# soedinglab/spacedust

Measured on AMD Instinct MI355X. Metric: clustersearch throughput (genome-pairs/s; SW GCUPS alongside), higher is better.
Workload: dtype int16

## Files before the change

### spacedust_amd/csrc/hip/sd_sw.hip

```cpp
#include "sd_common.h"
#include <unistd.h>


#include <algorithm>
#include <cmath>
#include <cstring>
#include <memory>
#include <omp.h>
#include <numeric>

#include "../host/sd_host.h"
#include "sd_sw_pk.h"

namespace {

using sdpk::SwTask;

template <int RT>
__global__ void __launch_bounds__(64)
sw_score_kernel(const SwTask *__restrict__ tasks, uint32_t nTasks, const uint8_t *__restrict__ qRes,
                const int8_t *__restrict__ qBias, const uint8_t *__restrict__ tRes, const int8_t *__restrict__ mat,
                int go, int ge, int32_t *__restrict__ out, uint2 *__restrict__ boundary,
                const uint32_t *__restrict__ order ,
                const int8_t *__restrict__ qProf ) {
// ... 1223 lines not shown
            uint32_t v = count;
            for (uint32_t d = 0; d < nd; d++) {
                *--o = (char) ('0' + v % 10);
                v /= 10;
            }
        }
        out += __shfl(incl, 63, 64);
        if (starts) runStart = base + (uint32_t) (63 - __clzll((long long) starts));
        left = __shfl(c, 63, 64);
    }
    if (lane == 0) {
        if (WRITE) {
            res[i].btOffset = dense[i];
            res[i].flags = (res[i].flags & 0xFF) | (int32_t) (out << 8);
        } else {
            cigLen[i] = out;
        }
    }
}

constexpr double BB_EVAL_EXACT = 1e-290;
struct BestByGroup {
    const uint32_t *groupOf, *groupKey;
    uint32_t nGroups;
    float seqIdThr, covThr;
    int alnLenThr, covMode;
    double evalThr;
    double evalExact;
};
__device__ __forceinline__ float bbCov(uint32_t startPos, uint32_t endPos, uint32_t len) {
    return (float) (min(len, max(startPos, endPos)) - min(startPos, endPos) + 1u) / (float) len;
}
__device__ __forceinline__ bool bbAccepted(const sd_sw_result &r, const BestByGroup &B, uint32_t qL, uint32_t tL) {
    if (r.btLen <= 0 || r.qStart < 0 || r.tStart < 0) return false;
    const float qcov = bbCov((uint32_t) r.qStart, (uint32_t) r.qEnd, qL), dbcov = bbCov((uint32_t) r.tStart, (uint32_t) r.tEnd, tL);
    const float seqId = (float) r.identical / (float) r.btLen;
    bool cov = true;
    if (B.covMode == 0) cov = qcov >= B.covThr && dbcov >= B.covThr;
    else if (B.covMode == 2) cov = qcov >= B.covThr;
    else if (B.covMode == 1) cov = dbcov >= B.covThr;
    return r.evalue <= B.evalThr * (1.0 + 1e-9) && seqId >= B.seqIdThr && cov && r.btLen >= B.alnLenThr;
}
__device__ __forceinline__ unsigned long long bbPack(const sd_sw_result &r, uint32_t tL, uint32_t key) {
    return ((unsigned long long) min((uint32_t) r.score, 0xFFFFFu) << 44) | ((unsigned long long) (0xFFFFu - min(tL, 0xFFFFu)) << 28) |
           (unsigned long long) (0x0FFFFFFFu - min(key, 0x0FFFFFFFu));
}
__global__ void __launch_bounds__(256)
k_best_mark(uint32_t nPairs, const sd_sw_result *__restrict__ res, const uint8_t *__restrict__ ident, const uint32_t *__restrict__ pq,
            const uint32_t *__restrict__ pt, const uint64_t *__restrict__ qOff, const uint64_t *__restrict__ tOff, BestByGroup B,
            unsigned long long *__restrict__ table) {
    const uint32_t i = blockIdx.x * blockDim.x + threadIdx.x;
    if (i >= nPairs || ident[i]) return;
    const uint32_t q = pq[i], t = pt[i];
    const uint32_t qL = (uint32_t) (qOff[q + 1] - qOff[q]), tL = (uint32_t) (tOff[t + 1] - tOff[t]);
    const sd_sw_result r = res[i];
    if (!bbAccepted(r, B, qL, tL)) return;
    atomicMax(&table[(size_t) q * B.nGroups + B.groupOf[t]], bbPack(r, tL, B.groupKey ? B.groupKey[t] : t));
}
__global__ void __launch_bounds__(256)
k_best_keep(uint32_t nPairs, sd_sw_result *__restrict__ res, const uint8_t *__restrict__ ident, const uint32_t *__restrict__ pq,
            const uint32_t *__restrict__ pt, const uint64_t *__restrict__ qOff, const uint64_t *__restrict__ tOff, BestByGroup B,
            const unsigned long long *__restrict__ table, uint64_t *__restrict__ btLen) {
    const uint32_t i = blockIdx.x * blockDim.x + threadIdx.x;
    if (i >= nPairs || ident[i]) return;
    const uint32_t q = pq[i], t = pt[i];
    const uint32_t qL = (uint32_t) (qOff[q + 1] - qOff[q]), tL = (uint32_t) (tOff[t + 1] - tOff[t]);
    const sd_sw_result r = res[i];
    const bool keep = bbAccepted(r, B, qL, tL) &&
                      (r.evalue < B.evalExact || table[(size_t) q * B.nGroups + B.groupOf[t]] == bbPack(r, tL, B.groupKey ? B.groupKey[t] : t));
    if (!keep) {
        res[i].btLen = 0;
        btLen[i] = 0;
    }
}

__global__ void __launch_bounds__(256)
k_accept(uint32_t nPairs, const sd_sw_result *__restrict__ res, const uint8_t *__restrict__ ident, uint8_t *__restrict__ acc) {
    const uint32_t i = blockIdx.x * blockDim.x + threadIdx.x;
    if (i >= nPairs) return;
    const sd_sw_result &r = res[i];
    acc[i] = (ident[i] || (r.btLen > 0 && r.qStart >= 0 && r.tStart >= 0)) ? 1 : 0;
}
__global__ void __launch_bounds__(256)
k_accept_compact(uint32_t nPairs, const sd_sw_result *__restrict__ res, const uint8_t *__restrict__ acc,
                 const uint64_t *__restrict__ pos, sd_sw_result *__restrict__ outRes, uint32_t *__restrict__ outIdx) {
    const uint32_t i = blockIdx.x * blockDim.x + threadIdx.x;
    if (i >= nPairs || !acc[i]) return;
    outRes[pos[i]] = res[i];
    outIdx[pos[i]] = i;
}
#include "sd_scan_sort.h"

template <typename T>
int devExclusiveScan(sd_ctx *ctx, const T *in, uint64_t *out, size_t n) {
    uint64_t *tmp = nullptr;
    SD_HIP(ctx, wsGet(ctx, "al.scantmp", sdScanTmpBytes(n) / sizeof(uint64_t) + 32, &tmp));
    SD_HIP(ctx, (sdScanLaunch<T, ScanSum64, false, uint64_t>(ctx->stream, in, out, n, tmp)));
    return SD_OK;
}
int devInclusiveMax(sd_ctx *ctx, const uint32_t *in, uint32_t *out, size_t n) {
    uint32_t *tmp = nullptr;
    SD_HIP(ctx, wsGet(ctx, "al.scantmp32", sdScanTmpBytes(n) / sizeof(uint32_t) + 32, &tmp));
    SD_HIP(ctx, (sdScanLaunch<uint32_t, ScanMax32, true, uint32_t>(ctx->stream, in, out, n, tmp)));
    return SD_OK;
}

int devSortPairs(sd_ctx *ctx, const uint32_t *kIn, uint32_t *kOut, const uint32_t *vIn, uint32_t *vOut, size_t n, int endBit) {
    if (n == 0) return SD_OK;
    uint32_t *kTmp = nullptr, *vTmp = nullptr, *cnt = nullptr;
    SD_HIP(ctx, wsGet(ctx, "al.sortK", n, &kTmp));
    SD_HIP(ctx, wsGet(ctx, "al.sortV", n, &vTmp));
    SD_HIP(ctx, wsGet(ctx, "al.sortCounts", sdRadixSortCountsBytes() / sizeof(uint32_t), &cnt));
    SD_HIP(ctx, sdRadixSortPairs(ctx->stream, kIn, vIn, kOut, vOut, kTmp, vTmp, (uint32_t) n, 0, endBit, cnt));
    return SD_OK;
}

__global__ void __launch_bounds__(256)
k_bound_need(uint32_t nPairs, const SwTask *__restrict__ tasks, const uint32_t *__restrict__ keys, uint64_t *__restrict__ need) {
    const uint32_t i = blockIdx.x * blockDim.x + threadIdx.x;
    if (i >= nPairs) return;
    uint64_t v = 0;
    if (keys[i] != KEY_INVALID) {
        const uint32_t ci = keys[i] >> 10;
        if (scoreClassIsMulti(ci)) v = 2ull * (uint64_t) tasks[i].tL;
        else if (ci == N_SCORE_CLASSES - 1 && tasks[i].n > 1024) v = (uint64_t) tasks[i].tL;
    }
    need[i] = v;
}
__global__ void __launch_bounds__(256)
k_bound_apply(uint32_t nPairs, SwTask *__restrict__ tasks, const uint64_t *__restrict__ off) {
    const uint32_t i = blockIdx.x * blockDim.x + threadIdx.x;
    if (i >= nPairs) return;
    tasks[i].boundOff = off[i];
}

constexpr uint32_t PAIR_NONE = 0xFFFFFFFFu;
inline bool sdSwQuads() {
    static const bool on = !(getenv("SD_SW_QUADS") && atoi(getenv("SD_SW_QUADS")) == 0);
    return on;
}
inline int sdSwWaves() {
    static const int w = (sdSwQuads() && getenv("SD_SW_WAVES") && atoi(getenv("SD_SW_WAVES")) == 2) ? 2 : 1;
    return w;
}
constexpr int PAIR_QUERY_BITS = 17;
__global__ void __launch_bounds__(256)
k_pair_keys(uint32_t n, const uint32_t *__restrict__ keys, const uint32_t *__restrict__ pairQ, uint32_t *__restrict__ key2) {
    const uint32_t i = blockIdx.x * blockDim.x + threadIdx.x;
    if (i >= n) return;
    const uint32_t k = keys[i];
    key2[i] = k == KEY_INVALID ? 0xFFFFFFFFu : ((k >> 10) << 26) | (pairQ[i] << 9) | ((k & 1023u) >> 1);
}
__global__ void __launch_bounds__(256)
k_pair_heads(uint32_t n, const uint32_t *__restrict__ keyS, uint32_t *__restrict__ headPos) {
    const uint32_t p = blockIdx.x * blockDim.x + threadIdx.x;
    if (p >= n) return;
    const bool head = p == 0 || (keyS[p] >> 9) != (keyS[p - 1] >> 9);
    headPos[p] = head ? p : 0u;
}
__global__ void __launch_bounds__(256)
k_pair_leaders(uint32_t n, const uint32_t *__restrict__ keyS, const uint32_t *__restrict__ runStart, uint8_t *__restrict__ leader, int quads) {
    const uint32_t p = blockIdx.x * blockDim.x + threadIdx.x;
    if (p > n) return;
    uint8_t v = 0;
    if (p < n && (keyS[p] >> 26) < FIRST_INT32_CLASS) {
        const uint32_t o = p - runStart[p];
        v = (o & 1u) == 0 ? 1 : 0;
        if (quads) {
            const bool lastOfRun = p + 1 >= n || (keyS[p + 1] >> 9) != (keyS[p] >> 9);
            const uint32_t pairs = (o + 1 + 1) / 2;
            if (lastOfRun) v += (uint8_t) (((uint32_t) quads - pairs % (uint32_t) quads) % (uint32_t) quads);
        }
    }
    leader[p] = v;
}
__global__ void __launch_bounds__(256)
k_pair_emit(uint32_t n, const uint32_t *__restrict__ keyS, const uint32_t *__restrict__ vals, const uint32_t *__restrict__ runStartOf,
            const uint64_t *__restrict__ pairIdx, uint32_t *__restrict__ order2) {
    const uint32_t p = blockIdx.x * blockDim.x + threadIdx.x;
    if (p >= n || (keyS[p] >> 26) >= FIRST_INT32_CLASS || ((p - runStartOf[p]) & 1u)) return;
    const uint64_t w = pairIdx[p];
    order2[2 * w] = vals[p];
    const bool mate = p + 1 < n && (keyS[p + 1] >> 9) == (keyS[p] >> 9);
    order2[2 * w + 1] = mate ? vals[p + 1] : PAIR_NONE;
}
__global__ void k_pair_bounds(const uint32_t *__restrict__ keyS, uint32_t n, const uint64_t *__restrict__ pairIdx,
                              uint32_t *__restrict__ b, int nb) {
    const int c = threadIdx.x;
    if (c >= nb) return;
    const uint32_t want = (uint32_t) c << 26;
    uint32_t lo = 0, hi = n;
    while (lo < hi) {
        const uint32_t mid = (lo + hi) >> 1;
        if (keyS[mid] < want) lo = mid + 1;
        else hi = mid;
    }
    b[c] = (uint32_t) pairIdx[lo];
}

int devRunScore(sd_ctx *ctx, uint32_t nPairs, const uint32_t *dKeys, const uint32_t *dVals, uint32_t *dKeysSorted,
                uint32_t *dOrder, uint32_t *dBounds, SwTask *dTasks, uint64_t *dScanA, uint64_t *dScanB,
                const sd_seqset *q, const sd_seqset *t, const int8_t *dMat, int go, int ge, int32_t *dOut,
                uint32_t *nValid, const uint32_t *dPairQ ) {
    const unsigned grid = (nPairs + 255) / 256;
    int rc = SD_OK;
    uint32_t *dOrder2 = nullptr, *dPairBounds = nullptr;
    if (dPairQ) {
        uint32_t *dKey2 = nullptr, *dVals2 = nullptr, *dHead = nullptr, *dRunStart = nullptr;
        uint64_t *dPairIdx = nullptr;
        uint8_t *dLeader = nullptr;
        SD_HIP(ctx, wsGet(ctx, "sp.key2", (size_t) nPairs, &dKey2));
        SD_HIP(ctx, wsGet(ctx, "sp.vals2", (size_t) nPairs, &dVals2));
        SD_HIP(ctx, wsGet(ctx, "sp.head", (size_t) nPairs, &dHead));
        SD_HIP(ctx, wsGet(ctx, "sp.runstart", (size_t) nPairs, &dRunStart));
        SD_HIP(ctx, wsGet(ctx, "sp.leader", (size_t) nPairs + 1, &dLeader));
        SD_HIP(ctx, wsGet(ctx, "sp.pairidx", (size_t) nPairs + 1, &dPairIdx));
        const int padPairs = sdSwQuads() ? 2 * sdSwWaves() : 0;
        const size_t order2Cap = (size_t) 2 * (size_t) std::max(padPairs, 2) * nPairs + 8;
        SD_HIP(ctx, wsGet(ctx, "sp.order2", order2Cap, &dOrder2));
        SD_HIP(ctx, hipMemsetAsync(dOrder2, 0xFF, order2Cap * sizeof(uint32_t), ctx->stream));
        SD_HIP(ctx, wsGet(ctx, "sp.bounds", 64, &dPairBounds));
        hipLaunchKernelGGL(k_pair_keys, dim3(grid), dim3(256), 0, ctx->stream, nPairs, dKeys, dPairQ, dKey2);
        rc = devSortPairs(ctx, dKey2, dKeysSorted, dVals, dVals2, nPairs, 32);
        if (rc != SD_OK) return rc;
        dOrder = dVals2;
        hipLaunchKernelGGL(k_pair_heads, dim3(grid), dim3(256), 0, ctx->stream, nPairs, dKeysSorted, dHead);
        rc = devInclusiveMax(ctx, dHead, dRunStart, nPairs);
        if (rc != SD_OK) return rc;
        hipLaunchKernelGGL(k_pair_leaders, dim3((nPairs + 256) / 256), dim3(256), 0, ctx->stream, nPairs, dKeysSorted, dRunStart, dLeader,
                           padPairs);
        rc = devExclusiveScan(ctx, (const uint8_t *) dLeader, dPairIdx, (size_t) nPairs + 1);
        if (rc != SD_OK) return rc;
        hipLaunchKernelGGL(k_pair_emit, dim3(grid), dim3(256), 0, ctx->stream, nPairs, dKeysSorted, dVals2, dRunStart, dPairIdx, dOrder2);
        hipLaunchKernelGGL(k_pair_bounds, dim3(1), dim3(64), 0, ctx->stream, dKeysSorted, nPairs, dPairIdx, dPairBounds,
                           (int) FIRST_INT32_CLASS + 1);
        hipLaunchKernelGGL(k_bounds, dim3(1), dim3(64), 0, ctx->stream, dKeysSorted, nPairs, 1u << 26, dBounds, (int) N_SCORE_CLASSES + 1);
    } else {
        rc = devSortPairs(ctx, dKeys, dKeysSorted, dVals, dOrder, nPairs, 16);
        if (rc != SD_OK) return rc;
        hipLaunchKernelGGL(k_bounds, dim3(1), dim3(64), 0, ctx->stream, dKeysSorted, nPairs, 1024u, dBounds, (int) N_SCORE_CLASSES + 1);
    }
    hipLaunchKernelGGL(k_bound_need, dim3(grid), dim3(256), 0, ctx->stream, nPairs, dTasks, dKeys, dScanA);
    SD_HIP(ctx, hipMemsetAsync(dScanA + nPairs, 0, sizeof(uint64_t), ctx->stream));
    rc = devExclusiveScan(ctx, dScanA, dScanB, (size_t) nPairs + 1);
    if (rc != SD_OK) return rc;
    hipLaunchKernelGGL(k_bound_apply, dim3(grid), dim3(256), 0, ctx->stream, nPairs, dTasks, dScanB);
    uint32_t hb[N_SCORE_CLASSES + 1], hpb[FIRST_INT32_CLASS + 1];
    uint64_t boundTotal = 0;
    if (dPairQ) SD_HIP(ctx, sdD2H(ctx, hpb, dPairBounds, sizeof(hpb)));
    SD_HIP(ctx, sdD2H(ctx, hb, dBounds, sizeof(hb)));
    SD_HIP(ctx, sdD2H(ctx, &boundTotal, dScanB + nPairs, sizeof(uint64_t)));
    SD_HIP(ctx, sdStreamSync(ctx));
    *nValid = hb[N_SCORE_CLASSES];
    uint2 *dBound = nullptr;
    SD_HIP(ctx, wsGet(ctx, "sw.bound", std::max<uint64_t>(boundTotal, 1), &dBound));
    for (uint32_t ci = 0; ci < N_SCORE_CLASSES; ci++) {
        const uint32_t begin = hb[ci], cnt = hb[ci + 1] - hb[ci];
        if (cnt == 0) continue;
        static const char *const pkNames[N_PK_CLASSES] = {"rt4x32", "rt6x32", "rt7x32", "rt8x32", "rt9x32", "rt10x32", "rt11x32", "rt12x32",
                                                          "rt8x64", "rt10x64", "rt12x64", "rt8x64s2", "rt8x64s3", "rt8x64sN"};
        static const char *const i32Names[4] = {"sw_score.rt4", "sw_score.rt8", "sw_score.rt16", "sw_score.rt32"};
        static const bool long32 = !(getenv("SD_SW_LONG32") && atoi(getenv("SD_SW_LONG32")) == 0);
        static const bool useAligned = !(getenv("SD_SW_ALIGNED") && atoi(getenv("SD_SW_ALIGNED")) == 0);
        const bool shared = dPairQ != nullptr && ci < FIRST_INT32_CLASS;
        const int alignedRT = (ci >= 1 && ci < FIRST_NARROW_MULTI) ? (int) ci + 4 : 0;
        const bool aligned = alignedRT > 0 && useAligned && (alignedRT <= 12 || (shared && long32));
        int generalIdx = 0;
        if (ci >= FIRST_NARROW_MULTI && ci < FIRST_WIDE_CLASS) generalIdx = (int) FIRST_MULTI_PK + (int) (ci - FIRST_NARROW_MULTI);
        else if (alignedRT) generalIdx = alignedRT <= 6 ? 1 : (alignedRT <= 12 ? alignedRT - 5 : (alignedRT <= 16 ? 8 : (alignedRT <= 20 ? 9 : 10)));
        char name[48];
        if (aligned) snprintf(name, sizeof(name), "sw_score_pk.a_seg%d", alignedRT);
        else if (ci < FIRST_WIDE_CLASS) snprintf(name, sizeof(name), "sw_score_pk.%s", pkNames[generalIdx]);
        else if (ci < FIRST_INT32_CLASS) snprintf(name, sizeof(name), "sw_score_pk.w_%s", pkNames[ci - FIRST_WIDE_CLASS]);
        else snprintf(name, sizeof(name), "%s", i32Names[ci - FIRST_INT32_CLASS]);
        ProfScope ps(ctx, name);
        const uint32_t *ord = dOrder + begin;
        uint32_t nOrd = cnt;
        if (shared) {
            ord = dOrder2 + 2 * (size_t) hpb[ci];
            nOrd = 2 * (hpb[ci + 1] - hpb[ci]);
        }
#define SD_PK(RT, LW, MULTI, WIDE)                                                                                          \
    do {                                                                                                                   \
        if (shared) launchScorePk<RT, LW, MULTI, WIDE, true>(ctx, dTasks, ord, nOrd, q, t, dMat, go, ge, dOut, dBound);     \
        else launchScorePk<RT, LW, MULTI, WIDE, false>(ctx, dTasks, ord, nOrd, q, t, dMat, go, ge, dOut, dBound);           \
    } while (0)
#define SD_PKA(RT)                                                                                               \
    case RT:                                                                                                     \
        if (shared && quads && sdSwWaves() == 2) launchScorePkAligned<RT, 32, 2, 2>(ctx, dTasks, ord, nOrd, q, t, dMat, go, ge, dOut);  \
        else if (shared && quads && sdSwChain() > 1) launchScorePkChain<RT>(ctx, dTasks, ord, nOrd, q, t, dMat, go, ge, dOut);  \
        else if (shared && quads) launchScorePkAligned<RT, 32, 2>(ctx, dTasks, ord, nOrd, q, t, dMat, go, ge, dOut);  \
        else if (shared) launchScorePkAligned<RT, 32, 1>(ctx, dTasks, ord, nOrd, q, t, dMat, go, ge, dOut);      \
        else launchScorePkAligned<RT, 32, 0>(ctx, dTasks, ord, nOrd, q, t, dMat, go, ge, dOut);                  \
        break;
#define SD_PKA16(SEG)                                                                                            \
    case SEG: launchScorePkAligned<2 * SEG, 16, 1>(ctx, dTasks, ord, nOrd, q, t, dMat, go, ge, dOut); break;
#define SD_PK_CLASS(WIDE, IDX)                                                \
        switch (IDX) {                                                        \
            case 0: SD_PK(4, 32, false, WIDE); break;                         \
            case 1: SD_PK(6, 32, false, WIDE); break;                         \
            case 2: SD_PK(7, 32, false, WIDE); break;                         \
            case 3: SD_PK(8, 32, false, WIDE); break;                         \
            case 4: SD_PK(9, 32, false, WIDE); break;                         \
            case 5: SD_PK(10, 32, false, WIDE); break;                        \
            case 6: SD_PK(11, 32, false, WIDE); break;                        \
            case 7: SD_PK(12, 32, false, WIDE); break;                        \
            case 8: SD_PK(8, 64, false, WIDE); break;                         \
            case 9: SD_PK(10, 64, false, WIDE); break;                        \
            case 10: SD_PK(12, 64, false, WIDE); break;                       \
            default: SD_PK(8, 64, true, WIDE); break;                         \
        }
        static const int lw16Max = getenv("SD_SW_LW16") ? atoi(getenv("SD_SW_LW16")) : (sdSwQuads() ? 0 : 8);
        const bool quads = sdSwQuads();
        if (aligned && shared && alignedRT <= lw16Max) {
            switch (alignedRT) {
                SD_PKA16(5) SD_PKA16(6) SD_PKA16(7) SD_PKA16(8) SD_PKA16(9) SD_PKA16(10) SD_PKA16(11) SD_PKA16(12)
                default: break;
            }
        } else if (aligned) {
            switch (alignedRT) {
                SD_PKA(5) SD_PKA(6) SD_PKA(7) SD_PKA(8) SD_PKA(9) SD_PKA(10) SD_PKA(11) SD_PKA(12) SD_PKA(13) SD_PKA(14)
                SD_PKA(15) SD_PKA(16) SD_PKA(17) SD_PKA(18) SD_PKA(19) SD_PKA(20) SD_PKA(21) SD_PKA(22) SD_PKA(23) SD_PKA(24)
                default: break;
            }
        } else if (ci < FIRST_WIDE_CLASS) {
            SD_PK_CLASS(false, generalIdx)
        } else if (ci < FIRST_INT32_CLASS) {
            SD_PK_CLASS(true, (int) (ci - FIRST_WIDE_CLASS))
        } else {
            switch (ci - FIRST_INT32_CLASS) {
                case 0: launchScoreIdx<4>(ctx, dTasks, ord, cnt, q, t, dMat, go, ge, dOut, dBound); break;
                case 1: launchScoreIdx<8>(ctx, dTasks, ord, cnt, q, t, dMat, go, ge, dOut, dBound); break;
                case 2: launchScoreIdx<16>(ctx, dTasks, ord, cnt, q, t, dMat, go, ge, dOut, dBound); break;
                default: launchScoreIdx<32>(ctx, dTasks, ord, cnt, q, t, dMat, go, ge, dOut, dBound); break;
            }
        }
#undef SD_PKA
#undef SD_PKA16
#undef SD_PK_CLASS
#undef SD_PK
    }
    SD_HIP(ctx, hipGetLastError());
    return SD_OK;
}

__global__ void __launch_bounds__(256)
k_cells(uint32_t nPairs, const SwTask *__restrict__ tasks, const uint32_t *__restrict__ keys, unsigned long long *__restrict__ acc) {
    const uint32_t i = blockIdx.x * blockDim.x + threadIdx.x;
    unsigned long long c = 0;
    if (i < nPairs && keys[i] != KEY_INVALID) c = (unsigned long long) tasks[i].n * (unsigned long long) tasks[i].tL;
#pragma unroll
    for (int off = 32; off >= 1; off >>= 1) c += __shfl_xor(c, off, 64);
    if ((threadIdx.x & 63) == 0 && c) atomicAdd(acc, c);
}

}

int sdFail(sd_ctx *ctx, int code, const char *fmt, ...) {
    char buf[1024];
    va_list ap;
    va_start(ap, fmt);
    vsnprintf(buf, sizeof(buf), fmt, ap);
    va_end(ap);
    if (ctx) ctx->lastError = buf;
    else fprintf(stderr, "spacedust_gpu: %s\n", buf);
    return code;
}

extern "C" {

int sd_ctx_create(int device, sd_ctx **out) { return sd_ctx_create_prio(device, 0, out); }

int sd_ctx_create_prio(int device, int priority, sd_ctx **out) { return sd_ctx_create_masked(device, priority, 0, out); }

int sd_ctx_create_masked(int device, int priority, int reserveCUs, sd_ctx **out) {
    if (out == nullptr) return SD_EINVAL;
    *out = nullptr;
    int count = 0;
    hipError_t e = hipGetDeviceCount(&count);
    if (e != hipSuccess || count <= 0) {
        fprintf(stderr, "spacedust_gpu: no HIP device visible (%s); this library has no CPU fallback\n",
                e != hipSuccess ? hipGetErrorString(e) : "device count 0");
        return SD_ENODEVICE;
    }
    if (device < 0 || device >= count) return SD_EINVAL;
    if (hipSetDevice(device) != hipSuccess) return SD_ENODEVICE;
    sd_ctx *c = new sd_ctx();
    c->device = device;
    int least = 0, greatest = 0;
    (void) hipDeviceGetStreamPriorityRange(&least, &greatest);
    const int prio = priority < 0 ? greatest : (priority > 0 ? least : (least + greatest) / 2);
    hipError_t se = hipSuccess;
    (void) hipGetDeviceProperties(&c->prop, device);
    const int nCU = c->prop.multiProcessorCount;
    if (reserveCUs > 0 && nCU > 0 && reserveCUs < nCU) {
        std::vector<uint32_t> mask((size_t) (nCU + 31) / 32, 0u);
        for (int b = 0; b < nCU - reserveCUs; b++) mask[(size_t) b / 32] |= 1u << (b % 32);
        se = hipExtStreamCreateWithCUMask(&c->stream, (uint32_t) mask.size(), mask.data());
    } else {
        se = hipStreamCreateWithPriority(&c->stream, hipStreamNonBlocking, prio);
    }
    if (se != hipSuccess) {
        delete c;
        return SD_EHIP;
    }
    const char *syncMode = getenv("SD_SYNC");
    const bool spin = syncMode && strcmp(syncMode, "spin") == 0;
    (void) hipEventCreate(&c->evStart);
    (void) hipEventCreate(&c->evStop);
    if (!spin) (void) hipEventCreateWithFlags(&c->evSync, hipEventDisableTiming);
    (void) hipGetDeviceProperties(&c->prop, device);
    *out = c;
    return SD_OK;
}

void sd_ctx_destroy(sd_ctx *ctx) {
    if (!ctx) return;
// ... 278 lines not shown
        }
        tk.segLen = std::max(1, (tk.n + lanes - 1) / lanes);
        tk.slot = i;
        tk.boundOff = 0;
        if (tk.n > 0 && tk.tL > 0) tasks.push_back(tk);
    }
    std::vector<int32_t> h;
    uint64_t cells = 0;
    int rc = runScoreTasks(ctx, tasks, queries, targets, dMat.p, par->gapOpen, par->gapExtend, h, nPairs, &cells);
    if (rc != SD_OK) return rc;
    if (reverse) ctx->cellsRev = cells; else ctx->cellsFwd = cells;
    for (uint32_t i = 0; i < nPairs; i++) {
        int v = h[3 * i], col = h[3 * i + 1], row = h[3 * i + 2];
        out[3 * i] = v;
        if (!reverse) {
            out[3 * i + 1] = col;
            out[3 * i + 2] = row;
        } else {
            out[3 * i + 1] = col < 0 ? -1 : tEnd[i] - col;
            out[3 * i + 2] = row;
        }
    }
    return SD_OK;
}

static int alignBatchImpl(sd_ctx *ctx, const sd_sw_params *par, const sd_seqset *queries, const sd_seqset *targets,
                          uint32_t nPairs, const uint32_t *pairQ, const uint32_t *pairT, const uint8_t *isIdentity,
                          sd_sw_result *out, char *btPool, uint64_t btCap, uint64_t *btUsed, uint32_t *compactIdx,
                          uint32_t *nCompact, const uint16_t *pairDiag = nullptr ,
                          const float *bestBy = nullptr ) {
    if (!ctx || !par || !queries || !targets || !out) return SD_EINVAL;
    if (compactIdx && (!nCompact || par->swMode != 2)) return sdFail(ctx, SD_EINVAL, "the compact variants need swMode 2 (records with backtraces)");
    (void) hipSetDevice(ctx->device);
    sdD2HReset(ctx);
    if (btUsed) *btUsed = 0;
    if (nCompact) *nCompact = 0;
    if (nPairs == 0) return SD_OK;
    const int go = par->gapOpen, ge = par->gapExtend;
    ctx->cellsFwd = ctx->cellsRev = ctx->cellsTb = 0;
    sd::Evaluer ev;
    sd::initEvaluer(ev, par->dbResidues);
    int matMin = 0;
    for (int i = 0; i < 441; i++) matMin = std::min(matMin, (int) par->matrix[i]);
    for (uint32_t i = 0; i < nPairs; i++)
        if (pairQ[i] >= queries->n || pairT[i] >= targets->n) return sdFail(ctx, SD_EINVAL, "pair %u out of range", i);
    if (targets->dProf) return sdFail(ctx, SD_EUNSUPPORTED, "profile targets are not implemented (profile queries are)");
    std::unique_ptr<HostScope> hs(new HostScope(ctx, "align.upload"));
    DevGateParams gp;
    gp.go = go; gp.ge = ge; gp.matMin = matMin; gp.swMode = par->swMode; gp.covMode = par->covMode; gp.covThr = par->covThr;
    {
        int matMax = 0;
        for (int x = 0; x < 441; x++) matMax = std::max(matMax, (int) par->matrix[x]);
        const int maxEntry = std::max(1, queries->dProf ? queries->maxEntryAdd : matMax + queries->maxEntryAdd);
        gp.wideRowLimit = 32767 / maxEntry;
    }
    gp.evalThr = par->evalThr;
    gp.lambda = ev.lambda; gp.K = ev.K; gp.aI = ev.aI; gp.bI = ev.bI; gp.alphaI = ev.alphaI; gp.betaI = ev.betaI;
    gp.aJ = ev.aJ; gp.bJ = ev.bJ; gp.alphaJ = ev.alphaJ; gp.betaJ = ev.betaJ; gp.sigma = ev.sigma; gp.tau = ev.tau;
    gp.viThr = ev.viThr; gp.vjThr = ev.vjThr; gp.cThr = ev.cThr; gp.dbResidues = ev.dbResidues;

    const size_t N = nPairs;
    const unsigned grid = (unsigned) ((N + 255) / 256);
    int8_t *dMat = nullptr;
    uint32_t *dPQ = nullptr, *dPT = nullptr, *dKeys = nullptr, *dVals = nullptr, *dKeysS = nullptr, *dOrder = nullptr,
             *dBounds = nullptr, *dFwdKeys = nullptr, *dRevKeys = nullptr;
    uint8_t *dIdent = nullptr, *dWord = nullptr;
    int32_t *dMinBias = nullptr, *dOut32 = nullptr, *dOut16 = nullptr, *dOutRev = nullptr, *dTbRes = nullptr;
    int *dErr = nullptr;
    SwTask *dTasks = nullptr;
    TbTask *dTb = nullptr;
    sd_sw_result *dRes = nullptr;
    uint64_t *dScanA = nullptr, *dScanB = nullptr, *dDirBytes = nullptr, *dDirOff = nullptr, *dBtBytes = nullptr,
             *dBtOff = nullptr, *dBtLen = nullptr, *dDense = nullptr;
    unsigned long long *dCells = nullptr;
    SD_HIP(ctx, wsGet(ctx, "al.mat", 448, &dMat));
    SD_HIP(ctx, wsGet(ctx, "al.pq", N, &dPQ));
    SD_HIP(ctx, wsGet(ctx, "al.pt", N, &dPT));
    SD_HIP(ctx, wsGet(ctx, "al.ident", N, &dIdent));
    SD_HIP(ctx, wsGet(ctx, "al.word", N, &dWord));
    SD_HIP(ctx, wsGet(ctx, "al.keys", N, &dKeys));
    SD_HIP(ctx, wsGet(ctx, "al.vals", N, &dVals));
    SD_HIP(ctx, wsGet(ctx, "al.keyss", N, &dKeysS));
    SD_HIP(ctx, wsGet(ctx, "al.order", N, &dOrder));
    SD_HIP(ctx, wsGet(ctx, "al.fwdkeys", N, &dFwdKeys));
    SD_HIP(ctx, wsGet(ctx, "al.revkeys", N, &dRevKeys));
    SD_HIP(ctx, wsGet(ctx, "al.bounds", 64, &dBounds));
    SD_HIP(ctx, wsGet(ctx, "al.minbias", queries->n, &dMinBias));
    SD_HIP(ctx, wsGet(ctx, "al.out32", N * 3, &dOut32));
    SD_HIP(ctx, wsGet(ctx, "al.out16", N * 3, &dOut16));
    SD_HIP(ctx, wsGet(ctx, "al.outrev", N * 3, &dOutRev));
    SD_HIP(ctx, wsGet(ctx, "al.tbres", N * 2, &dTbRes));
    SD_HIP(ctx, wsGet(ctx, "al.err", 4, &dErr));
    SD_HIP(ctx, wsGet(ctx, "al.tasks", N, &dTasks));
    SD_HIP(ctx, wsGet(ctx, "al.tb", N, &dTb));
    SD_HIP(ctx, wsGet(ctx, "al.res", N, &dRes));
    SD_HIP(ctx, wsGet(ctx, "al.scana", N + 1, &dScanA));
    SD_HIP(ctx, wsGet(ctx, "al.scanb", N + 1, &dScanB));
    SD_HIP(ctx, wsGet(ctx, "al.dirbytes", N + 1, &dDirBytes));
    SD_HIP(ctx, wsGet(ctx, "al.diroff", N + 1, &dDirOff));
    SD_HIP(ctx, wsGet(ctx, "al.btbytes", N + 1, &dBtBytes));
    SD_HIP(ctx, wsGet(ctx, "al.btoff", N + 1, &dBtOff));
    SD_HIP(ctx, wsGet(ctx, "al.btlen", N + 1, &dBtLen));
    SD_HIP(ctx, wsGet(ctx, "al.dense", N + 1, &dDense));
    SD_HIP(ctx, wsGet(ctx, "al.cells", 4, &dCells));
    SD_HIP(ctx, hipMemcpyAsync(dMat, par->matrix, 441, hipMemcpyHostToDevice, ctx->stream));
    SD_HIP(ctx, hipMemcpyAsync(dPQ, pairQ, N * sizeof(uint32_t), hipMemcpyHostToDevice, ctx->stream));
    SD_HIP(ctx, hipMemcpyAsync(dPT, pairT, N * sizeof(uint32_t), hipMemcpyHostToDevice, ctx->stream));
    if (isIdentity) SD_HIP(ctx, hipMemcpyAsync(dIdent, isIdentity, N, hipMemcpyHostToDevice, ctx->stream));
    else SD_HIP(ctx, hipMemsetAsync(dIdent, 0, N, ctx->stream));
    SD_HIP(ctx, hipMemcpyAsync(dMinBias, queries->dProf ? queries->hProfBias.data() : queries->hMinBias.data(),
                               queries->n * sizeof(int32_t), hipMemcpyHostToDevice, ctx->stream));
    SD_HIP(ctx, hipMemsetAsync(dErr, 0, 4 * sizeof(int), ctx->stream));
    SD_HIP(ctx, hipMemsetAsync(dCells, 0, 4 * sizeof(unsigned long long), ctx->stream));
    SD_HIP(ctx, hipMemsetAsync(dOut32, 0, N * 3 * sizeof(int32_t), ctx->stream));
    SD_HIP(ctx, hipMemsetAsync(dOut16, 0, N * 3 * sizeof(int32_t), ctx->stream));
    SD_HIP(ctx, hipMemsetAsync(dOutRev, 0, N * 3 * sizeof(int32_t), ctx->stream));
    SD_HIP(ctx, hipMemsetAsync(dBtLen, 0, (N + 1) * sizeof(uint64_t), ctx->stream));

    hs.reset(new HostScope(ctx, "align.fwd32"));
    const int usePk = (go >= ge && go < 1024 && ge >= 0 && getenv("SD_SW_INT32") == nullptr) ? 1 : 0;
    uint32_t nValid = 0;
    hipLaunchKernelGGL(k_make_fwd, dim3(grid), dim3(256), 0, ctx->stream, nPairs, dPQ, dPT, dIdent, queries->dOff, targets->dOff,
                       dTasks, dFwdKeys, dVals, dRes, usePk);
    uint32_t *dPass1Keys = dFwdKeys;
    uint8_t *dPreWord = nullptr;
    if (pairDiag && usePk && !getenv("SD_SW_NO_PREWORD")) {
        uint16_t *dDiag = nullptr;
        SD_HIP(ctx, wsGet(ctx, "al.diag", N, &dDiag));
        SD_HIP(ctx, wsGet(ctx, "al.preword", N, &dPreWord));
        SD_HIP(ctx, wsGet(ctx, "al.pass1keys", N, &dPass1Keys));
        SD_HIP(ctx, hipMemcpyAsync(dDiag, pairDiag, N * sizeof(uint16_t), hipMemcpyHostToDevice, ctx->stream));
        hipLaunchKernelGGL(k_pre_word, dim3(grid), dim3(256), 0, ctx->stream, nPairs, (const uint32_t *) dPQ, (const uint32_t *) dPT,
                           (const uint16_t *) dDiag, (const uint32_t *) dFwdKeys, (const uint64_t *) queries->dOff, (const uint64_t *) targets->dOff,
                           (const uint8_t *) queries->dRes, (const int8_t *) queries->dBias, (const uint8_t *) targets->dRes, (const int8_t *) dMat,
                           (const int8_t *) queries->dProf, (const int32_t *) dMinBias, queries->dProf ? 0 : matMin, dPreWord, dPass1Keys);
    }
    hipLaunchKernelGGL(k_cells, dim3(grid), dim3(256), 0, ctx->stream, nPairs, dTasks, dPass1Keys, dCells + 0);
    const uint32_t *dShare = (getenv("SD_SW_NOSHARE") || queries->n >= (1u << PAIR_QUERY_BITS)) ? nullptr : dPQ;
    int rc = devRunScore(ctx, nPairs, dPass1Keys, dVals, dKeysS, dOrder, dBounds, dTasks, dScanA, dScanB, queries, targets, dMat, go,
                         ge, dOut32, &nValid, dShare);
    if (rc != SD_OK) return rc;
    hs.reset(new HostScope(ctx, "align.fwd16"));
    hipLaunchKernelGGL(k_gate_word, dim3(grid), dim3(256), 0, ctx->stream, nPairs, dPQ, dOut32, dMinBias, queries->dProf ? 0 : matMin, dTasks, dKeys,
                       dVals, dWord, dFwdKeys, usePk, gp.wideRowLimit, (const uint8_t *) dPreWord);
    hipLaunchKernelGGL(k_cells, dim3(grid), dim3(256), 0, ctx->stream, nPairs, dTasks, dKeys, dCells + 0);
    rc = devRunScore(ctx, nPairs, dKeys, dVals, dKeysS, dOrder, dBounds, dTasks, dScanA, dScanB, queries, targets, dMat, go, ge,
                     dOut16, &nValid, dShare);
    if (rc != SD_OK) return rc;
    hs.reset(new HostScope(ctx, "align.rev"));
    hipLaunchKernelGGL(k_gate_rev, dim3(grid), dim3(256), 0, ctx->stream, nPairs, gp, dPQ, dPT, queries->dOff, targets->dOff, dOut32,
                       dOut16, dWord, dFwdKeys, dTasks, dRevKeys, dVals, dRes, usePk);
    hipLaunchKernelGGL(k_cells, dim3(grid), dim3(256), 0, ctx->stream, nPairs, dTasks, dRevKeys, dCells + 1);
    rc = devRunScore(ctx, nPairs, dRevKeys, dVals, dKeysS, dOrder, dBounds, dTasks, dScanA, dScanB, queries, targets, dMat, go, ge,
                     dOutRev, &nValid, nullptr);
    if (rc != SD_OK) return rc;
    hs.reset(new HostScope(ctx, "align.traceback"));
    hipLaunchKernelGGL(k_gate_tb, dim3(grid), dim3(256), 0, ctx->stream, nPairs, gp, dPQ, dPT, queries->dOff, targets->dOff, dOutRev,
                       dRevKeys, dTb, dKeys, dVals, dDirBytes, dBtBytes, dRes, dErr);
    SD_HIP(ctx, hipMemsetAsync(dBtBytes + N, 0, sizeof(uint64_t), ctx->stream));
    rc = devExclusiveScan(ctx, dBtBytes, dBtOff, N + 1);
    if (rc != SD_OK) return rc;
    uint64_t btScratch = 0;
    SD_HIP(ctx, sdD2H(ctx, &btScratch, dBtOff + N, sizeof(uint64_t)));
    SD_HIP(ctx, sdStreamSync(ctx));
    char *dBt = nullptr;
    SD_HIP(ctx, wsGet(ctx, "tb.bt", btScratch + 64, &dBt));
    uint64_t SCRATCH_BUDGET = 16ull << 30;
    {
        size_t freeB = 0, totalB = 0;
        if (hipMemGetInfo(&freeB, &totalB) == hipSuccess && totalB > 0)
            SCRATCH_BUDGET = std::max<uint64_t>(1ull << 30, std::min<uint64_t>(totalB / 4, freeB / 3));
        if (const char *e = getenv("SD_TB_BUDGET")) SCRATCH_BUDGET = std::max<uint64_t>(1u << 20, strtoull(e, nullptr, 10));
    }
    uint32_t *dKeysRound = nullptr;
    SD_HIP(ctx, wsGet(ctx, "tb.keysRound", N + 1, &dKeysRound));
    bool tbPending = false, budgetRaised = false;
    for (int round = 0; round < 4096; round++) {
        tbPending = true;
        SD_HIP(ctx, hipMemsetAsync(dDirBytes + N, 0, sizeof(uint64_t), ctx->stream));
        rc = devExclusiveScan(ctx, dDirBytes, dDirOff, N + 1);
        if (rc != SD_OK) return rc;
        hipLaunchKernelGGL(k_tb_round, dim3(grid), dim3(256), 0, ctx->stream, nPairs, dKeys, dDirOff, dDirBytes, SCRATCH_BUDGET, dKeysRound);
        hipLaunchKernelGGL(k_tb_offsets, dim3(grid), dim3(256), 0, ctx->stream, nPairs, dKeysRound, dDirOff, dBtOff, dTb);
        rc = devSortPairs(ctx, dKeysRound, dKeysS, dVals, dOrder, nPairs, 16);
        if (rc != SD_OK) return rc;
        hipLaunchKernelGGL(k_bounds, dim3(1), dim3(64), 0, ctx->stream, dKeysS, nPairs, 4096u, dBounds, (int) N_TB_CLASSES + 1);
        uint32_t hb[N_TB_CLASSES + 1];
        uint64_t dirTotal = 0;
        SD_HIP(ctx, sdD2H(ctx, hb, dBounds, sizeof(hb)));
        SD_HIP(ctx, sdD2H(ctx, &dirTotal, dDirOff + N, sizeof(uint64_t)));
        SD_HIP(ctx, sdStreamSync(ctx));
        if (hb[N_TB_CLASSES] == 0) {
            if (dirTotal == 0) {
                tbPending = false;
                break;
            }
            if (SCRATCH_BUDGET >= dirTotal) return sdFail(ctx, SD_EHIP, "traceback: pending tasks but an empty round (budget %llu, pending %llu bytes)",
                                                          (unsigned long long) SCRATCH_BUDGET, (unsigned long long) dirTotal);
            SCRATCH_BUDGET = std::min<uint64_t>(dirTotal, SCRATCH_BUDGET * 2);
            budgetRaised = true;
            continue;
        }
        if (getenv("SD_DEBUG_TB")) {
            fprintf(stderr, "[tb] round %d: narrow", round);
            for (int ci = 0; ci < N_TB_NARROW; ci++) fprintf(stderr, " %u", hb[ci + 1] - hb[ci]);
            fprintf(stderr, " lds %u %u %u global %u dir %.1f MB\n", hb[N_TB_NARROW + 1] - hb[N_TB_NARROW], hb[N_TB_NARROW + 2] - hb[N_TB_NARROW + 1],
                    hb[N_TB_NARROW + 3] - hb[N_TB_NARROW + 2], hb[N_TB_NARROW + 4] - hb[N_TB_NARROW + 3], dirTotal / 1e6);
        }
        int8_t *dDir = nullptr;
        if (wsGet(ctx, "tb.dir", std::min<uint64_t>(dirTotal, SCRATCH_BUDGET) + 64, &dDir) != hipSuccess) {
            (void) hipGetLastError();
            if (SCRATCH_BUDGET <= (256ull << 20) || budgetRaised)
                return sdFail(ctx, SD_ENOMEM, "traceback direction scratch: out of device memory (%llu bytes for one round)",
                              (unsigned long long) std::min<uint64_t>(dirTotal, SCRATCH_BUDGET));
            SCRATCH_BUDGET /= 2;
            continue;
        }
        for (int ci = 0; ci < N_TB_NARROW; ci++) {
            const uint32_t begin = hb[ci], cnt = hb[ci + 1] - hb[ci];
            if (cnt == 0) continue;
            static const char *const tbNames[N_TB_NARROW] = {"sw_traceback.narrow128", "sw_traceback.narrow192", "sw_traceback.narrow256",
                                                             "sw_traceback.narrow320", "sw_traceback.narrow384", "sw_traceback.narrow512",
                                                             "sw_traceback.narrow640", "sw_traceback.narrow768", "sw_traceback.narrow1024"};
            ProfScope ps(ctx, tbNames[ci]);
            const int qCap = TB_NARROW_Q[ci], tCap = qCap + 16;
            const size_t ldsBytes = 2 * ((size_t) 16 * qCap + 2 * (size_t) qCap + tCap);
            if (queries->dProf)
                hipLaunchKernelGGL(sw_traceback_narrow_kernel<true>, dim3((cnt + 1) / 2), dim3(64), ldsBytes, ctx->stream, dTb, cnt,
                                   queries->dRes, queries->dBias, targets->dRes, dMat, go, ge, qCap, tCap, dBt, dTbRes, dOrder + begin,
                                   (const int8_t *) queries->dProf);
            else
                hipLaunchKernelGGL(sw_traceback_narrow_kernel<false>, dim3((cnt + 1) / 2), dim3(64), ldsBytes, ctx->stream, dTb, cnt,
                                   queries->dRes, queries->dBias, targets->dRes, dMat, go, ge, qCap, tCap, dBt, dTbRes, dOrder + begin,
                                   (const int8_t *) nullptr);
        }
        static const int ldsClass[3] = {128, 512, 2048};
        for (int ci = 0; ci < 3; ci++) {
            const uint32_t begin = hb[N_TB_NARROW + ci], cnt = hb[N_TB_NARROW + 1 + ci] - hb[N_TB_NARROW + ci];
            if (cnt == 0) continue;
            ProfScope ps(ctx, "sw_traceback.lds");
            const int ldsStride = ldsClass[ci] + 1;
            const size_t ldsBytes = (size_t) 2 * 3 * ldsStride * sizeof(int32_t);
            if (queries->dProf)
                hipLaunchKernelGGL(sw_traceback_kernel<true>, dim3((cnt + 1) / 2), dim3(64), ldsBytes, ctx->stream, dTb, cnt, queries->dRes,
                                   queries->dBias, targets->dRes, dMat, go, ge, ldsStride, dDir, dBt, dTbRes, dOrder + begin,
                                   ldsClass[ci] - 1, (const int8_t *) queries->dProf);
            else
                hipLaunchKernelGGL(sw_traceback_kernel<false>, dim3((cnt + 1) / 2), dim3(64), ldsBytes, ctx->stream, dTb, cnt, queries->dRes,
                                   queries->dBias, targets->dRes, dMat, go, ge, ldsStride, dDir, dBt, dTbRes, dOrder + begin,
                                   ldsClass[ci] - 1, (const int8_t *) nullptr);
            hipLaunchKernelGGL(sw_traceback_walk_kernel<false>, dim3((cnt + 256 / TBW_LANES - 1) / (256 / TBW_LANES)), dim3(256), 0, ctx->stream, dTb, cnt, queries->dRes,
                               targets->dRes, dDir, dBt, dTbRes, dOrder + begin);
        }
        {
            const uint32_t begin = hb[N_TB_NARROW + 3], cnt = hb[N_TB_NARROW + 4] - hb[N_TB_NARROW + 3];
            if (cnt) {
                ProfScope ps(ctx, "sw_traceback.global");
                if (queries->dProf)
                    hipLaunchKernelGGL((sw_traceback_kernel<true, true>), dim3((cnt + 1) / 2), dim3(64), 0, ctx->stream, dTb, cnt, queries->dRes,
                                       queries->dBias, targets->dRes, dMat, go, ge, INT_MAX, dDir, dBt, dTbRes, dOrder + begin, 0,
                                       (const int8_t *) queries->dProf);
                else
                    hipLaunchKernelGGL((sw_traceback_kernel<false, true>), dim3((cnt + 1) / 2), dim3(64), 0, ctx->stream, dTb, cnt, queries->dRes,
                                       queries->dBias, targets->dRes, dMat, go, ge, INT_MAX, dDir, dBt, dTbRes, dOrder + begin, 0,
                                       (const int8_t *) nullptr);
                hipLaunchKernelGGL(sw_traceback_walk_kernel<true>, dim3((cnt + 256 / TBW_LANES - 1) / (256 / TBW_LANES)), dim3(256), 0, ctx->stream, dTb, cnt, queries->dRes,
                                   targets->dRes, dDir, dBt, dTbRes, dOrder + begin);
            }
        }
        SD_HIP(ctx, hipGetLastError());
        hipLaunchKernelGGL(k_tb_collect, dim3(grid), dim3(256), 0, ctx->stream, nPairs, dKeys, dVals, dTb, dTbRes, dDirBytes, dBtLen,
                           dRes, dErr, 4 * 65536, dKeysRound);
    }
    if (tbPending) return sdFail(ctx, SD_EHIP, "traceback: tasks still pending after 4096 rounds");
    if (getenv("SD_DEBUG_TB")) {
        std::vector<TbTask> hT(nPairs);
        std::vector<uint64_t> hL(nPairs);
        SD_HIP(ctx, hipMemcpy(hT.data(), dTb, (size_t) nPairs * sizeof(TbTask), hipMemcpyDeviceToHost));
        SD_HIP(ctx, hipMemcpy(hL.data(), dBtLen, (size_t) nPairs * sizeof(uint64_t), hipMemcpyDeviceToHost));
        uint64_t nDone = 0, init6 = 0, init6final6 = 0, init6final14 = 0, final14 = 0;
        for (uint32_t i = 0; i < nPairs; i++) {
            if (hL[i] == 0) continue;
            nDone++;
            const int ib = abs(hT[i].tLen - hT[i].qLen) + 1, fb = hT[i].band;
            if (ib <= 6) { init6++; if (fb <= 6) init6final6++; else if (fb <= 14) init6final14++; }
            if (fb <= 14) final14++;
        }
        {
            static const int lim[8] = {1, 2, 3, 4, 6, 8, 14, 1 << 30};
            uint64_t hi[8] = {0}, hf[8] = {0}, rowsF[8] = {0};
            for (uint32_t i = 0; i < nPairs; i++) {
                if (hL[i] == 0) continue;
                const int ib = abs(hT[i].tLen - hT[i].qLen) + 1, fb = hT[i].band;
                int a = 0, b = 0;
                while (ib > lim[a]) a++;
                while (fb > lim[b]) b++;
                hi[a]++;
                hf[b]++;
                rowsF[b] += (uint64_t) hT[i].qLen;
            }
            fprintf(stderr, "[tb] band <=1 <=2 <=3 <=4 <=6 <=8 <=14 >14: initial");
            for (int x = 0; x < 8; x++) fprintf(stderr, " %llu", (unsigned long long) hi[x]);
            fprintf(stderr, " | final");
            for (int x = 0; x < 8; x++) fprintf(stderr, " %llu", (unsigned long long) hf[x]);
            fprintf(stderr, " | rows by final");
            for (int x = 0; x < 8; x++) fprintf(stderr, " %llu", (unsigned long long) rowsF[x]);
            fprintf(stderr, "\n");
// ... 524 lines not shown
```

Measured before the change: 2779.

## Enable query-shared pair scheduling for the reverse alignment pass

Extends the shared-query pairing path to the reverse Smith-Waterman pass. A new key kernel builds composite keys from score class, query index and truncated query length, and a run-shift parameter generalizes run detection so pairs are grouped only when the whole key matches. Pairs that share a query can then reuse that query's data in the packed kernels. The cost is an extra sort and key-building pass on the reverse path, and multi classes are excluded from sharing.

```diff
diff --git a/spacedust_amd/csrc/hip/sd_sw.hip b/spacedust_amd/csrc/hip/sd_sw.hip
--- a/spacedust_amd/csrc/hip/sd_sw.hip
+++ b/spacedust_amd/csrc/hip/sd_sw.hip
@@ -1399,14 +1399,28 @@
     key2[i] = k == KEY_INVALID ? 0xFFFFFFFFu : ((k >> 10) << 26) | (pairQ[i] << 9) | ((k & 1023u) >> 1);
 }
 __global__ void __launch_bounds__(256)
-k_pair_heads(uint32_t n, const uint32_t *__restrict__ keyS, uint32_t *__restrict__ headPos) {
+k_pair_keys_rev(uint32_t n, const uint32_t *__restrict__ keysS, const uint32_t *__restrict__ perm, const uint32_t *__restrict__ pairQ,
+                const SwTask *__restrict__ tasks, uint32_t *__restrict__ key2) {
     const uint32_t p = blockIdx.x * blockDim.x + threadIdx.x;
     if (p >= n) return;
-    const bool head = p == 0 || (keyS[p] >> 9) != (keyS[p - 1] >> 9);
+    const uint32_t k = keysS[p];
+    if (k == KEY_INVALID) {
+        key2[p] = 0xFFFFFFFFu;
+        return;
+    }
+    const uint32_t i = perm[p];
+    key2[p] = ((k >> 10) << 26) | (pairQ[i] << 9) | ((uint32_t) (tasks[i].n - 1) & 511u);
+}
+__global__ void __launch_bounds__(256)
+k_pair_heads(uint32_t n, const uint32_t *__restrict__ keyS, uint32_t *__restrict__ headPos, int runShift) {
+    const uint32_t p = blockIdx.x * blockDim.x + threadIdx.x;
+    if (p >= n) return;
+    const bool head = p == 0 || (keyS[p] >> runShift) != (keyS[p - 1] >> runShift);
     headPos[p] = head ? p : 0u;
 }
 __global__ void __launch_bounds__(256)
-k_pair_leaders(uint32_t n, const uint32_t *__restrict__ keyS, const uint32_t *__restrict__ runStart, uint8_t *__restrict__ leader, int quads) {
+k_pair_leaders(uint32_t n, const uint32_t *__restrict__ keyS, const uint32_t *__restrict__ runStart, uint8_t *__restrict__ leader, int quads,
+               int runShift) {
     const uint32_t p = blockIdx.x * blockDim.x + threadIdx.x;
     if (p > n) return;
     uint8_t v = 0;
@@ -1414,7 +1428,7 @@
         const uint32_t o = p - runStart[p];
         v = (o & 1u) == 0 ? 1 : 0;
         if (quads) {
-            const bool lastOfRun = p + 1 >= n || (keyS[p + 1] >> 9) != (keyS[p] >> 9);
+            const bool lastOfRun = p + 1 >= n || (keyS[p + 1] >> runShift) != (keyS[p] >> runShift);
             const uint32_t pairs = (o + 1 + 1) / 2;
             if (lastOfRun) v += (uint8_t) (((uint32_t) quads - pairs % (uint32_t) quads) % (uint32_t) quads);
         }
@@ -1423,12 +1437,12 @@
 }
 __global__ void __launch_bounds__(256)
 k_pair_emit(uint32_t n, const uint32_t *__restrict__ keyS, const uint32_t *__restrict__ vals, const uint32_t *__restrict__ runStartOf,
-            const uint64_t *__restrict__ pairIdx, uint32_t *__restrict__ order2) {
+            const uint64_t *__restrict__ pairIdx, uint32_t *__restrict__ order2, int runShift) {
     const uint32_t p = blockIdx.x * blockDim.x + threadIdx.x;
     if (p >= n || (keyS[p] >> 26) >= FIRST_INT32_CLASS || ((p - runStartOf[p]) & 1u)) return;
     const uint64_t w = pairIdx[p];
     order2[2 * w] = vals[p];
-    const bool mate = p + 1 < n && (keyS[p + 1] >> 9) == (keyS[p] >> 9);
+    const bool mate = p + 1 < n && (keyS[p + 1] >> runShift) == (keyS[p] >> runShift);
     order2[2 * w + 1] = mate ? vals[p + 1] : PAIR_NONE;
 }
 __global__ void k_pair_bounds(const uint32_t *__restrict__ keyS, uint32_t n, const uint64_t *__restrict__ pairIdx,
@@ -1448,9 +1462,11 @@
 int devRunScore(sd_ctx *ctx, uint32_t nPairs, const uint32_t *dKeys, const uint32_t *dVals, uint32_t *dKeysSorted,
                 uint32_t *dOrder, uint32_t *dBounds, SwTask *dTasks, uint64_t *dScanA, uint64_t *dScanB,
                 const sd_seqset *q, const sd_seqset *t, const int8_t *dMat, int go, int ge, int32_t *dOut,
-                uint32_t *nValid, const uint32_t *dPairQ ) {
+                uint32_t *nValid, const uint32_t *dPairQ ,
+                bool revPairs = false ) {
     const unsigned grid = (nPairs + 255) / 256;
     int rc = SD_OK;
+    const int runShift = revPairs ? 0 : 9;
     uint32_t *dOrder2 = nullptr, *dPairBounds = nullptr;
     if (dPairQ) {
         uint32_t *dKey2 = nullptr, *dVals2 = nullptr, *dHead = nullptr, *dRunStart = nullptr;
@@ -1467,18 +1483,26 @@
         SD_HIP(ctx, wsGet(ctx, "sp.order2", order2Cap, &dOrder2));
         SD_HIP(ctx, hipMemsetAsync(dOrder2, 0xFF, order2Cap * sizeof(uint32_t), ctx->stream));
         SD_HIP(ctx, wsGet(ctx, "sp.bounds", 64, &dPairBounds));
-        hipLaunchKernelGGL(k_pair_keys, dim3(grid), dim3(256), 0, ctx->stream, nPairs, dKeys, dPairQ, dKey2);
-        rc = devSortPairs(ctx, dKey2, dKeysSorted, dVals, dVals2, nPairs, 32);
+        if (revPairs) {
+            rc = devSortPairs(ctx, dKeys, dKeysSorted, dVals, dOrder, nPairs, 16);
+            if (rc != SD_OK) return rc;
+            hipLaunchKernelGGL(k_pair_keys_rev, dim3(grid), dim3(256), 0, ctx->stream, nPairs, dKeysSorted, dOrder, dPairQ, dTasks, dKey2);
+            rc = devSortPairs(ctx, dKey2, dKeysSorted, dOrder, dVals2, nPairs, 32);
+        } else {
+            hipLaunchKernelGGL(k_pair_keys, dim3(grid), dim3(256), 0, ctx->stream, nPairs, dKeys, dPairQ, dKey2);
+            rc = devSortPairs(ctx, dKey2, dKeysSorted, dVals, dVals2, nPairs, 32);
+        }
         if (rc != SD_OK) return rc;
         dOrder = dVals2;
-        hipLaunchKernelGGL(k_pair_heads, dim3(grid), dim3(256), 0, ctx->stream, nPairs, dKeysSorted, dHead);
+        hipLaunchKernelGGL(k_pair_heads, dim3(grid), dim3(256), 0, ctx->stream, nPairs, dKeysSorted, dHead, runShift);
         rc = devInclusiveMax(ctx, dHead, dRunStart, nPairs);
         if (rc != SD_OK) return rc;
         hipLaunchKernelGGL(k_pair_leaders, dim3((nPairs + 256) / 256), dim3(256), 0, ctx->stream, nPairs, dKeysSorted, dRunStart, dLeader,
-                           padPairs);
+                           padPairs, runShift);
         rc = devExclusiveScan(ctx, (const uint8_t *) dLeader, dPairIdx, (size_t) nPairs + 1);
         if (rc != SD_OK) return rc;
-        hipLaunchKernelGGL(k_pair_emit, dim3(grid), dim3(256), 0, ctx->stream, nPairs, dKeysSorted, dVals2, dRunStart, dPairIdx, dOrder2);
+        hipLaunchKernelGGL(k_pair_emit, dim3(grid), dim3(256), 0, ctx->stream, nPairs, dKeysSorted, dVals2, dRunStart, dPairIdx, dOrder2,
+                           runShift);
         hipLaunchKernelGGL(k_pair_bounds, dim3(1), dim3(64), 0, ctx->stream, dKeysSorted, nPairs, dPairIdx, dPairBounds,
                            (int) FIRST_INT32_CLASS + 1);
         hipLaunchKernelGGL(k_bounds, dim3(1), dim3(64), 0, ctx->stream, dKeysSorted, nPairs, 1u << 26, dBounds, (int) N_SCORE_CLASSES + 1);
@@ -1509,7 +1533,7 @@
         static const char *const i32Names[4] = {"sw_score.rt4", "sw_score.rt8", "sw_score.rt16", "sw_score.rt32"};
         static const bool long32 = !(getenv("SD_SW_LONG32") && atoi(getenv("SD_SW_LONG32")) == 0);
         static const bool useAligned = !(getenv("SD_SW_ALIGNED") && atoi(getenv("SD_SW_ALIGNED")) == 0);
-        const bool shared = dPairQ != nullptr && ci < FIRST_INT32_CLASS;
+        const bool shared = dPairQ != nullptr && ci < FIRST_INT32_CLASS && !(revPairs && scoreClassIsMulti(ci));
         const int alignedRT = (ci >= 1 && ci < FIRST_NARROW_MULTI) ? (int) ci + 4 : 0;
         const bool aligned = alignedRT > 0 && useAligned && (alignedRT <= 12 || (shared && long32));
         int generalIdx = 0;
@@ -2094,7 +2118,7 @@
                        dOut16, dWord, dFwdKeys, dTasks, dRevKeys, dVals, dRes, usePk);
     hipLaunchKernelGGL(k_cells, dim3(grid), dim3(256), 0, ctx->stream, nPairs, dTasks, dRevKeys, dCells + 1);
     rc = devRunScore(ctx, nPairs, dRevKeys, dVals, dKeysS, dOrder, dBounds, dTasks, dScanA, dScanB, queries, targets, dMat, go, ge,
-                     dOutRev, &nValid, nullptr);
+                     dOutRev, &nValid, dShare, true);
     if (rc != SD_OK) return rc;
     hs.reset(new HostScope(ctx, "align.traceback"));
     hipLaunchKernelGGL(k_gate_tb, dim3(grid), dim3(256), 0, ctx->stream, nPairs, gp, dPQ, dPT, queries->dOff, targets->dOff, dOutRev,
```

After: 2803, median of 6. No clear change (+0.9%).
